# AbrahamSanders/realtime-codec-agent

Measured on NVIDIA B200. Metric: encode audio-sec/sec, higher is better.
Workload: dtype bf16

## Files before the change

realtime-codec-agent_b200/csrc/elementwise.cuh:

```cuda
#pragma once
#include "gemm_sm100.cuh"

namespace mc {

template <int KT>
__global__ void __launch_bounds__(256)
conv_first_kernel(const float* __restrict__ wav, long long ld, int T, int B, int T0, int s0, int C0,
                  const float* __restrict__ w , const float* __restrict__ bias,
                  __nv_bfloat16* __restrict__ out, int pad_rows) {
  pdl_launch_dependents();
  pdl_wait();
  const int cgroups = C0 / 8;
  const int cg = threadIdx.x % cgroups;
  const int slot = threadIdx.x / cgroups;
  const int frames_per_block = blockDim.x / cgroups;
  float wr[KT][8], br[8];
#pragma unroll
  for (int j = 0; j < KT; ++j) {
    const float4 a = __ldg(reinterpret_cast<const float4*>(w + j * C0 + cg * 8));
    const float4 c = __ldg(reinterpret_cast<const float4*>(w + j * C0 + cg * 8 + 4));
    wr[j][0] = a.x; wr[j][1] = a.y; wr[j][2] = a.z; wr[j][3] = a.w;
    wr[j][4] = c.x; wr[j][5] = c.y; wr[j][6] = c.z; wr[j][7] = c.w;
  }
#pragma unroll
// ... 78 lines not shown
#pragma unroll
    for (int u = 0; u < NV; ++u) ss += v[u].x * v[u].x + v[u].y * v[u].y + v[u].z * v[u].z + v[u].w * v[u].w;
#pragma unroll
    for (int o = 16; o > 0; o >>= 1) ss += __shfl_xor_sync(0xffffffffu, ss, o);
    const float inv = rsqrtf(ss / static_cast<float>(d) + eps);
    const int grp = row / grp_in;
    const long long obase = static_cast<long long>(grp) * grp_stride + grp_off + static_cast<long long>(row - grp * grp_in) * d;
    uint2* orow_p = reinterpret_cast<uint2*>(out + obase);
#pragma unroll
    for (int u = 0; u < NV; ++u) {
      uint2 o;
      o.x = pack_bf16x2(v[u].x * inv * g[u].x, v[u].y * inv * g[u].y);
      o.y = pack_bf16x2(v[u].z * inv * g[u].z, v[u].w * inv * g[u].w);
      orow_p[lane + 32 * u] = o;
    }
  }
}

__global__ void compact_rows_kernel(const float4* __restrict__ x, float4* __restrict__ y, int B, int r_in, int r_out,
                                    int d4) {
  pdl_launch_dependents();
  pdl_wait();
  const long long total = static_cast<long long>(B) * r_out * d4;
  for (long long idx = blockIdx.x * static_cast<long long>(blockDim.x) + threadIdx.x; idx < total;
       idx += static_cast<long long>(gridDim.x) * blockDim.x) {
    const int c = static_cast<int>(idx % d4);
    const long long row = idx / d4;
    const int j = static_cast<int>(row % r_out);
    const long long b = row / r_out;
    y[idx] = x[(b * r_in + (r_in - r_out) + j) * d4 + c];
  }
}

__global__ void gather_stem_kernel(const float4* __restrict__ stem, float4* __restrict__ x, int B, int F, int pre,
                                   int fstep, int d4) {
  pdl_launch_dependents();
  pdl_wait();
  const int per = F - pre;
  const long long total = static_cast<long long>(B) * per * d4;
  for (long long idx = blockIdx.x * static_cast<long long>(blockDim.x) + threadIdx.x; idx < total;
       idx += static_cast<long long>(gridDim.x) * blockDim.x) {
    const int c = static_cast<int>(idx % d4);
    const long long row = idx / d4;
    const int t = pre + static_cast<int>(row % per);
    const long long b = row / per;
    x[(b * F + t) * d4 + c] = __ldg(stem + (b * fstep + t) * d4 + c);
  }
}

__global__ void embed_codes_kernel(const long long* __restrict__ codes, const float* __restrict__ table ,
                                   int K, __nv_bfloat16* __restrict__ out, long long M) {
  pdl_launch_dependents();
  pdl_wait();
  const long long total = M * 8;
  for (long long idx = blockIdx.x * static_cast<long long>(blockDim.x) + threadIdx.x; idx < total;
       idx += static_cast<long long>(gridDim.x) * blockDim.x) {
    const long long m = idx >> 3;
    const int piece = static_cast<int>(idx & 7);
    uint4 o = make_uint4(0, 0, 0, 0);
    if (piece < 2) {
      long long code = codes[m];
      code = code < 0 ? 0 : (code >= K ? K - 1 : code);
      const float4* src = reinterpret_cast<const float4*>(table + code * 16 + piece * 8);
      const float4 a = __ldg(src), b = __ldg(src + 1);
      o.x = pack_bf16x2(a.x, a.y);
      o.y = pack_bf16x2(a.z, a.w);
      o.z = pack_bf16x2(b.x, b.y);
      o.w = pack_bf16x2(b.z, b.w);
    }
    *reinterpret_cast<uint4*>(out + m * 64 + piece * 8) = o;
  }
}

__global__ void pack_latents_kernel(const float* __restrict__ z , __nv_bfloat16* __restrict__ out,
                                    long long M) {
  const long long total = M * 8;
  for (long long idx = blockIdx.x * static_cast<long long>(blockDim.x) + threadIdx.x; idx < total;
       idx += static_cast<long long>(gridDim.x) * blockDim.x) {
    const long long m = idx >> 3;
// ... 129 lines not shown
```

realtime-codec-agent_b200/csrc/engine.cu:

```cuda
#include "engine_common.cuh"

#include "attn_sm100.cuh"
#include "attn_vq_simt.cuh"
#include "elementwise.cuh"
#include "gemm_sm100.cuh"
#include "gemm_splitk_sm100.cuh"
#include "ingest.cuh"
#include "post_sm100.cuh"
#include "vq_sm100.cuh"

using namespace mc;
using namespace mc_internal;

namespace {

struct GemmCall {
  const bf16* A; int64_t a_rows; int a_k_wrap;
  const bf16* W; const float* bias;
  int M, N, K, act, out_mode;
  void* out; int64_t ldo;
  int grp_in = INT_MAX, grp_valid = INT_MAX; int64_t grp_stride = 0, grp_off = 0;
  int rope_cols = 0, rope_period = 0, rope_offset = 0;
  int block_n = 0;
  const void* prefetch_ptr = nullptr;
// ... 238 lines not shown
  attention_window_simt_kernel<<<(unsigned)blocks, threads, 0, stream>>>(qkv, out, B, F, s.n_heads, s.window_left,
                                                                         s.window_right, out_rows, 0.125f);
  MC_LAUNCH_CHECK(h, "attention_window_simt_kernel");
  return MC_OK;
}

struct StackBufs {
  float* x;
  float* x2;
  bf16* hbuf;
  bf16* qkv;
  bf16* att;
  bf16* ffn;
  float* stats;
};

bool few_rows_regime(const mc_handle* h, long long M) {
  return (h->split_k == 2 || (h->split_k == 1 && h->in_session)) && M <= 2 * GEMM_BM;
}
bool fuse_norm_ok(const mc_handle* h, long long M) {
  if (h->spec.d_model % 64 != 0 || h->fuse_norm == 0) return false;
  return h->fuse_norm >= 2 || few_rows_regime(h, M);
}

int launch_rowstats(mc_handle* h, const float* x, const float* gamma, bf16* xb, float* stats, long long M, int d, cudaStream_t stream) {
  McProfScope prof(h, 3, 0.0, (double)M * d * 6.0, stream);
  mc_launch(h, rowstats_cast_kernel, dim3(ew_grid(h, M * (d / 64), 256)), dim3(256), 0, stream, x, gamma, xb, stats, M, d);
  MC_LAUNCH_CHECK(h, "rowstats_cast_kernel");
  return MC_OK;
}

int run_layers(mc_handle* h, const char* prefix, int n_layers, const StackBufs& b, int B, int F, int keep_rows,
               float** x_out, cudaStream_t stream, int fuse_mode = 0 ,
               const float* final_gamma = nullptr, bf16** xb_out = nullptr, float** stats_out = nullptr) {
  const mc_spec& s = h->spec;
  const int d = s.d_model, f = s.ffn_dim;
  const int nst = d / 64;
  const bool fused = fuse_mode == 1;
  const bool fused2 = fuse_mode != 0;
  std::vector<int> r_in(n_layers), r_out(n_layers);
  {
    int need = std::max(1, std::min(keep_rows, F));
    if (B == 1 && F <= GEMM_BM) need = F;
    for (int l = n_layers - 1; l >= 0; --l) {
      r_out[l] = need;
      need = (need >= F) ? F : std::min(F, need + s.window_left);
      if (!h->exact_cut && need < F) need = F - ((F - need) / 16) * 16;
      r_in[l] = need;
    }
  }
  float* x = b.x;
  float* xalt = b.x2;
  int rows = F;
  char name[128];
  for (int l = 0; l < n_layers; ++l) {
    auto T = [&](const char* leaf) {
      snprintf(name, sizeof(name), "%s.layers.%d.%s", prefix, l, leaf);
      return std::string(name);
    };
    const int Ri = rows, Ro = std::min(r_out[l], rows);
    const int Mi = B * Ri, Mo = B * Ro;
    if (!fused) MC_TRY(launch_rmsnorm(h, x, h->ptr<float>(T("norm1")), b.hbuf, Mi, d, INT_MAX, 0, 0, stream));
    GemmCall g{};
    if (fused) { g.row_stats = b.stats; g.row_stats_n = nst; }
    g.A = b.hbuf; g.a_rows = Mi; g.a_k_wrap = d; g.W = h->ptr<bf16>(T("wqkv")); g.bias = h->ptr<float>(T("bqkv"));
    g.M = Mi; g.N = 3 * d; g.K = d; g.act = ACT_NONE; g.out_mode = OUT_BF16; g.out = b.qkv; g.ldo = 3 * d;
    g.rope_cols = 2 * d; g.rope_period = Ri; g.rope_offset = F - Ri;
    g.prefetch_ptr = h->ptr<bf16>(T("wo")); g.prefetch_bytes = (long long)d * d * 2;
    MC_TRY(launch_gemm(h, g, stream));
    MC_TRY(launch_attention(h, b.qkv, b.att, B, Ri, Ro, (F - Ri) % 16, h->attn_impl, stream));
    if (Ro < Ri) {
      const long long items = (long long)Mo * (d / 4);
      McProfScope prof(h, 3, 0.0, (double)Mo * d * 8.0, stream);
      mc_launch(h, compact_rows_kernel, dim3(ew_grid(h, items, 256)), dim3(256), 0, stream, reinterpret_cast<const float4*>(x),
                reinterpret_cast<float4*>(xalt), B, Ri, Ro, d / 4);
      MC_LAUNCH_CHECK(h, "compact_rows_kernel");
      std::swap(x, xalt);
      rows = Ro;
    }
    GemmCall o{};
    o.A = b.att; o.a_rows = Mo; o.a_k_wrap = d; o.W = h->ptr<bf16>(T("wo")); o.bias = h->ptr<float>(T("bo"));
    o.M = Mo; o.N = d; o.K = d; o.act = ACT_NONE; o.out_mode = OUT_F32_RESIDUAL; o.out = x; o.ldo = d;
    o.prefetch_ptr = h->ptr<bf16>(T("w1")); o.prefetch_bytes = (long long)f * d * 2;
    if (fused2) { o.xb_out = b.hbuf; o.xb_gamma = h->ptr<float>(T("norm2")); o.stat_out = b.stats; }
    MC_TRY(launch_gemm(h, o, stream));
    if (!fused2) MC_TRY(launch_rmsnorm(h, x, h->ptr<float>(T("norm2")), b.hbuf, Mo, d, INT_MAX, 0, 0, stream));
    GemmCall u{};
    if (fused2) { u.row_stats = b.stats; u.row_stats_n = nst; }
    u.A = b.hbuf; u.a_rows = Mo; u.a_k_wrap = d; u.W = h->ptr<bf16>(T("w1")); u.bias = h->ptr<float>(T("b1"));
    u.M = Mo; u.N = f; u.K = d; u.act = ACT_GELU_TANH; u.out_mode = OUT_BF16; u.out = b.ffn; u.ldo = f;
    u.prefetch_ptr = h->ptr<bf16>(T("w2")); u.prefetch_bytes = (long long)d * f * 2;
    MC_TRY(launch_gemm(h, u, stream));
    GemmCall w{};
    w.A = b.ffn; w.a_rows = Mo; w.a_k_wrap = f; w.W = h->ptr<bf16>(T("w2")); w.bias = h->ptr<float>(T("b2"));
    w.M = Mo; w.N = d; w.K = f; w.act = ACT_NONE; w.out_mode = OUT_F32_RESIDUAL; w.out = x; w.ldo = d;
    if (l + 1 < n_layers) {
      snprintf(name, sizeof(name), "%s.layers.%d.wqkv", prefix, l + 1);
      w.prefetch_ptr = h->ptr<bf16>(name); w.prefetch_bytes = (long long)3 * d * d * 2;
    }
    if (fused) {
      const float* next_gamma = final_gamma;
      if (l + 1 < n_layers) {
// ... 140 lines not shown
  }
  return (int)dirty;
}

struct RaggedKeep {
  const int* rtable;
  int C, keep;
};

int encode_impl(mc_handle* h, const float* wav, int64_t ld, int B, int T, int keep, int64_t* codes, float* margin,
                float* z_e_out, cudaStream_t stream, const RaggedKeep* ragged = nullptr) {
  const mc_spec& s = h->spec;
  const int n = s.n_convs;
  int hop = 1;
  for (int i = 0; i < n; ++i) hop *= s.conv_strides[i];
  const int F = (T + hop - 1) / hop;
  if (F < 1) return h->fail(MC_ERR_ARG, "encode: empty input");
  if (F > s.max_positions) return h->fail(MC_ERR_ARG, "encode: %d frames exceed RoPE table (%d rows)", F, s.max_positions);
  if (keep <= 0 || keep > F) keep = F;
  const int Tp = F * hop;
  const int d = s.d_model, dq = s.codebook_dim;
  const long long Mll = (long long)B * F;
  if (Mll * std::max(3 * d, s.ffn_dim) > (long long)INT_MAX) return h->fail(MC_ERR_ARG, "encode: batch too large");
  const int M = (int)Mll;

  const int pre = stem_prefix_frames(s);
  const long long span_samples = (long long)(B - 1) * ld + T;
  const long long span_frames = span_samples / hop;
  const bool shared = h->shared_stem && B >= 2 && ld > 0 && ld < T && ld % hop == 0 && T % hop == 0 && F > pre &&
                      span_samples <= INT_MAX && span_frames + (long long)pre * B < (long long)B * F / 2;
  const int fuse_mode = !(fuse_norm_ok(h, Mll + B) && s.enc_layers > 0) ? 0 : ((h->fuse_norm == 3 && !few_rows_regime(h, Mll + B)) ? 2 : 1);
  const bool fused = fuse_mode == 1;
  const bool conv_producer = fused && few_rows_regime(h, Mll + B) && !shared;

  Carver cv;
  ConvPlan cp_full, cp_span, cp_pre;
  size_t ostem = 0;
  if (shared) {
    cp_span = plan_conv(s, cv, 1, (int)span_samples);
    cp_pre = plan_conv(s, cv, B, pre * hop);
    ostem = cv.take((size_t)span_frames * d * 4);
  } else {
    cp_full = plan_conv(s, cv, B, Tp);
  }
  Carver cv2 = cv;
  carve_stack(cv2, nullptr, M, d, s.ffn_dim, true);
  size_t oz = cv2.take((size_t)M * dq * 4);
  size_t ovq = cv2.take(vq_scratch_bytes(h, B * keep));
  const size_t ozg = ragged ? cv2.take((size_t)B * ragged->keep * dq * 4) : 0;
  MC_TRY(arena_reserve(h, cv2.off, stream));
  uint8_t* base = h->arena;
  StackBufs sb = carve_stack(cv, base, M, d, s.ffn_dim, false);
  float* z_e = reinterpret_cast<float*>(base + oz);
  void* vq_scratch = base + ovq;

  if (shared) {
    float* stem = reinterpret_cast<float*>(base + ostem);
    MC_TRY(run_conv_stack(h, cp_span, base, wav, span_samples, (int)span_samples, stem, 0, stream));
    MC_TRY(run_conv_stack(h, cp_pre, base, wav, ld, pre * hop, sb.x, (int64_t)F * d, stream));
    const long long items = (long long)B * (F - pre) * (d / 4);
    McProfScope prof(h, 3, 0.0, (double)B * (F - pre) * d * 8.0, stream);
    mc_launch(h, gather_stem_kernel, dim3(ew_grid(h, items, 256)), dim3(256), 0, stream, reinterpret_cast<const float4*>(stem),
              reinterpret_cast<float4*>(sb.x), B, F, pre, (int)(ld / hop), d / 4);
    MC_LAUNCH_CHECK(h, "gather_stem_kernel");
  } else {
    if (conv_producer)
      MC_TRY(run_conv_stack(h, cp_full, base, wav, ld, T, sb.x, (int64_t)F * d, stream, sb.hbuf, h->ptr<float>("enc.layers.0.norm1"), sb.stats));
    else
      MC_TRY(run_conv_stack(h, cp_full, base, wav, ld, T, sb.x, (int64_t)F * d, stream));
  }
  if (fused && !conv_producer) MC_TRY(launch_rowstats(h, sb.x, h->ptr<float>("enc.layers.0.norm1"), sb.hbuf, sb.stats, M, d, stream));
  const int keep_rows = z_e_out ? F : keep;
  float* xk = nullptr;
  bf16* xbk = sb.hbuf;
  float* stk = nullptr;
  MC_TRY(run_layers(h, "enc", s.enc_layers, sb, B, F, keep_rows, &xk, stream, fuse_mode, fused ? h->ptr<float>("enc.norm_f") : nullptr, &xbk, &stk));
  const int Mk = B * keep_rows;
  if (!fused) MC_TRY(launch_rmsnorm(h, xk, h->ptr<float>("enc.norm_f"), sb.hbuf, Mk, d, INT_MAX, 0, 0, stream));
  GemmCall pj{};
  if (fused) { pj.row_stats = stk; pj.row_stats_n = d / 64; }
  pj.A = fused ? xbk : sb.hbuf; pj.a_rows = Mk; pj.a_k_wrap = d; pj.W = h->ptr<bf16>("enc.proj.w"); pj.bias = h->ptr<float>("enc.proj.b");
  pj.M = Mk; pj.N = dq; pj.K = d; pj.act = ACT_NONE; pj.out_mode = OUT_F32; pj.out = z_e; pj.ldo = dq;
  MC_TRY(launch_gemm(h, pj, stream));
  if (z_e_out) MC_CUDA(h, cudaMemcpyAsync(z_e_out, z_e, (size_t)M * dq * 4, cudaMemcpyDeviceToDevice, stream));
  if (ragged) {
    float* zg = reinterpret_cast<float*>(base + ozg);
    pool_gather_rows_ragged_kernel<<<dim3(1, B), 256, 0, stream>>>(z_e, ragged->rtable, ragged->C, keep_rows, F, ragged->keep,
                                                                   dq, hop, zg);
    MC_LAUNCH_CHECK(h, "pool_gather_rows_ragged_kernel");
    return launch_vq(h, zg, B, ragged->keep, ragged->keep, codes, margin, vq_scratch, stream);
  }
  MC_TRY(launch_vq(h, z_e, B, keep_rows, keep, codes, margin, vq_scratch, stream));
  return MC_OK;
}

int decode_impl(mc_handle* h, const int64_t* codes, const float* z_q, int B, int F, int keep, float* wav,
                cudaStream_t stream) {
  const mc_spec& s = h->spec;
  const int n = s.n_convs;
  if (F < 1 || B < 1) return h->fail(MC_ERR_ARG, "decode: empty input");
  if (F > s.max_positions) return h->fail(MC_ERR_ARG, "decode: %d frames exceed RoPE table (%d rows)", F, s.max_positions);
  int hop = 1;
  for (int i = 0; i < n; ++i) hop *= s.conv_strides[i];
  const int d = s.d_model;
  const long long Mll = (long long)B * F;
  if (Mll * std::max(3 * d, s.ffn_dim) > (long long)INT_MAX) return h->fail(MC_ERR_ARG, "decode: batch too large");
  const int M = (int)Mll;
  const int total = F * hop;
  if (keep <= 0 || keep > total) keep = total;
// ... 338 lines not shown
}

int64_t mc_launch_count(const mc_handle* h) { return h ? h->launches : 0; }

int mc_profile_begin(mc_handle* h) {
  if (!h) return MC_ERR_ARG;
  for (auto& r : h->prof) { h->event_pool.push_back(r.a); h->event_pool.push_back(r.b); }
  h->prof.clear();
  h->profiling = true;
  return MC_OK;
}

int mc_profile_end(mc_handle* h, double* ms, double* flops, double* bytes, int64_t* launches, int32_t n_classes) {
  if (!h || !ms || !flops || !bytes || !launches) return MC_ERR_ARG;
  h->profiling = false;
  for (int c = 0; c < n_classes; ++c) { ms[c] = 0; flops[c] = 0; bytes[c] = 0; launches[c] = 0; }
  for (auto& r : h->prof) {
    cudaError_t e = cudaEventSynchronize(r.b);
    if (e != cudaSuccess) return h->fail(MC_ERR_CUDA, "mc_profile_end: %s", cudaGetErrorString(e));
    float t = 0.f;
    cudaEventElapsedTime(&t, r.a, r.b);
    if (r.cls < n_classes) { ms[r.cls] += t; flops[r.cls] += r.flops; bytes[r.cls] += r.bytes; launches[r.cls]++; }
    h->event_pool.push_back(r.a); h->event_pool.push_back(r.b);
  }
  h->prof.clear();
  return MC_OK;
}

int mc_set_option(mc_handle* h, const char* key, int32_t value) {
  if (!h || !key) return MC_ERR_ARG;
  const std::string k(key);
  if (k == "shared_stem") h->shared_stem = value != 0;
  else if (k == "exact_cut") { h->exact_cut = value != 0; h->tensor_gen++; }
  else if (k == "gemm_pair") h->gemm_pair = value != 0;
  else if (k == "fast_epilogue") h->fast_epilogue = value != 0;
  else if (k == "pdl") h->pdl = value != 0;
  else if (k == "attn_p_tmem") h->attn_p_tmem = value != 0;
  else if (k == "debug_repeat") h->debug_repeat = value;
  else if (k == "l2_prefetch") { h->l2_prefetch = value != 0; h->tensor_gen++; }
  else if (k == "fuse_norm") {
    if (value < 0 || value > 3) return h->fail(MC_ERR_ARG, "mc_set_option: fuse_norm is 0 .. 3");
    h->fuse_norm = value; h->tensor_gen++;
  }
  else if (k == "small_m_split_k") {
    if (value < 0 || value > 2) return h->fail(MC_ERR_ARG, "mc_set_option: small_m_split_k is 0, 1 or 2");
    h->split_k = value;
    h->tensor_gen++;
  }
  else if (k == "max_positions") {
    if (value < 1) return h->fail(MC_ERR_ARG, "mc_set_option: max_positions must be positive");
    h->spec.max_positions = value;
  }
  else return h->fail(MC_ERR_ARG, "mc_set_option: unknown option '%s'", key);
  return MC_OK;
}

int mc_set_debug_impl(mc_handle* h, int32_t attention_impl, int32_t vq_impl) {
  if (!h) return MC_ERR_ARG;
  h->gemm_pair = (attention_impl & 4) ? 0 : 1;
  attention_impl &= 1;
  h->attn_impl = attention_impl;
  h->vq_impl = vq_impl;
  return MC_OK;
}

int mc_op_gemm(mc_handle* h, const void* A, int64_t a_rows, int32_t a_k_wrap, const void* W, const float* bias,
// ... 909 lines not shown
```

realtime-codec-agent_b200/csrc/engine_common.cuh:

```cuda
#pragma once
#include <cuda.h>
#include <cuda_runtime.h>
#include <stdarg.h>
#include <stdio.h>
#include <string.h>

#include <algorithm>
#include <climits>
#include <map>
#include <set>
#include <string>
#include <tuple>
#include <unordered_map>
#include <utility>
#include <vector>

#include "../../include/magicodec_b200.h"
#include "ptx_sm100.cuh"

typedef __nv_bfloat16 bf16;

namespace mc_internal {

inline thread_local std::string g_create_error;
// ... 14 lines not shown
  }
  return fn;
}

struct Tensor {
  const void* p = nullptr;
  int64_t numel = 0;
};

}
using mc_internal::Tensor;

struct mc_handle {
  mc_spec spec{};
  int device = 0;
  int num_sms = 148;
  bool finalized = false;
  std::unordered_map<std::string, Tensor> tensors;
  std::string err;
  int64_t launches = 0;
  uint32_t tensor_gen = 0;
  int attn_impl = 0, vq_impl = 0;
  int gemm_pair = 1;
  bool fast_epilogue = true;
  bool attn_p_tmem = true;
  int split_k = 1;
  bool in_session = false;
  int debug_repeat = 1;
  int fuse_norm = 1;
  bool l2_prefetch = true;
  bool pdl = true;
  bool shared_stem = true;
  bool exact_cut = true;
  struct ProfRec { cudaEvent_t a, b; int cls; double flops; double bytes; };
  bool profiling = false;
  std::vector<ProfRec> prof;
  std::vector<cudaEvent_t> event_pool;
  std::set<const void*> smem_configured;
  uint8_t* arena = nullptr;
  size_t arena_cap = 0;
  size_t arena_off = 0;
  std::map<std::tuple<const void*, uint64_t, uint64_t, uint64_t, uint32_t, uint32_t>, CUtensorMap> maps;

  int fail(int code, const char* fmt, ...) {
    char buf[1024];
    va_list ap;
    va_start(ap, fmt);
    vsnprintf(buf, sizeof(buf), fmt, ap);
    va_end(ap);
    err = buf;
    return code;
  }
  const Tensor* find(const std::string& name) const {
    auto it = tensors.find(name);
    return it == tensors.end() ? nullptr : &it->second;
  }
  template <typename T>
  const T* ptr(const std::string& name) const {
    return reinterpret_cast<const T*>(tensors.at(name).p);
  }
};

#define MC_CUDA(h, expr)                                                                         \
  do {                                                                                           \
    cudaError_t e__ = (expr);                                                                    \
    if (e__ != cudaSuccess)                                                                      \
// ... 113 lines not shown
```

realtime-codec-agent_b200/csrc/gemm_sm100.cuh:

```cuda
#pragma once
#include <type_traits>

#include "ptx_sm100.cuh"

namespace mc {

enum : int { ACT_NONE = 0, ACT_GELU_TANH = 1 };
enum : int { OUT_BF16 = 0, OUT_F32 = 1, OUT_F32_RESIDUAL = 2 };

struct GemmParams {
  int M, N, K;
  int a_k_wrap;
  const float* bias;
  int act;
  int out_mode;
  void* out;
  long long ldo;
  int grp_in, grp_valid;
  long long grp_stride, grp_off;
  int tma_store;
  const float* rope_cos;
  int rope_ld;
  const float* rope_sin;
  int rope_cols;
// ... 26 lines not shown

constexpr int GEMM_BM = 128;
constexpr int GEMM_BK = 64;
constexpr int GEMM_THREADS = 256;
constexpr int kEpiBufBytes = 4096;

template <int BN>
struct GemmCfg {
  static constexpr int kStageBytesA = GEMM_BM * GEMM_BK * 2;
  static constexpr int kStageBytesB = BN * GEMM_BK * 2;
  static constexpr int kStageBytes = kStageBytesA + kStageBytesB;
  static constexpr int kStages = (BN == 256) ? 4 : (BN == 128 ? 6 : 8);
  static constexpr int kTmemCols = 2 * BN;
  static constexpr int kEpiBytes = 4 * 2 * kEpiBufBytes;
  static constexpr int kBarBytes = 256;
  static constexpr int kSmemBytes = kStages * kStageBytes + kEpiBytes + kBarBytes + 1024;
};

__device__ __forceinline__ float gelu_tanh_f(float x) {
  const float x2 = x * x;
  const float inner = fmaf(x2, 0.7978845608028654f * 0.044715f, 0.7978845608028654f);
  const float u = x * inner;
  float t;
  asm("tanh.approx.f32 %0, %1;" : "=f"(t) : "f"(u));
  const float hx = 0.5f * x;
  return fmaf(hx, t, hx);
}

__device__ __forceinline__ uint32_t pack_bf16x2(float lo, float hi) {
  __nv_bfloat162 h = __floats2bfloat162_rn(lo, hi);
  return *reinterpret_cast<uint32_t*>(&h);
}

struct EpiRegs {
  float bias[64];
  float rc[32], rs[32];
  int rope_pos = -1;
  int buf_sel = 0;
};

template <int BN>
__device__ __forceinline__ void epi_load_bias(const GemmParams& p, int n0, float (&b)[64]) {
#pragma unroll
  for (int j = 0; j < 64; j += 4) {
    float4 b4 = make_float4(0.f, 0.f, 0.f, 0.f);
    if (n0 + j < p.N) b4 = __ldg(reinterpret_cast<const float4*>(p.bias + n0 + j));
    b[j] = b4.x; b[j + 1] = b4.y; b[j + 2] = b4.z; b[j + 3] = b4.w;
  }
}

template <int BN, int RPW = 32>
__device__ __forceinline__ void gemm_epilogue_slab(const GemmParams& p, const CUtensorMap* map_out_p, uint32_t tmem_acc,
                                                   int row_base, int n_base, int q, int lane, uint8_t* my_bufs,
                                                   EpiRegs& st, uint64_t* ready_bar, uint32_t ready_parity) {
  const int g = row_base + q * RPW + (lane < RPW ? lane : 0);
  const int grp = g / p.grp_in;
  const int r = g - grp * p.grp_in;
  const bool row_ok = (lane < RPW) && (g < p.M) && (r < p.grp_valid);
  const long long obase = static_cast<long long>(grp) * p.grp_stride + p.grp_off + static_cast<long long>(r) * p.ldo;
  const bool has_bias = p.bias != nullptr;
  if (has_bias) epi_load_bias<BN>(p, n_base, st.bias);
  const float rs = (p.row_stats != nullptr && g < p.M) ? row_rs(p, g) : 1.0f;
  if (p.rope_period > 0) {
    const int pos = p.rope_offset + r % p.rope_period;
    if (pos != st.rope_pos) {
      st.rope_pos = pos;
// ... 10 lines not shown
#pragma unroll 1
  for (int c = 0; c < BN / 64; ++c) {
    const int n0 = n_base + c * 64;
    if (n0 >= p.N) break;
    uint32_t raw0[32], raw1[32];
    const uint32_t taddr = tmem_acc + (static_cast<uint32_t>(q * 32) << 16) + c * 64;
    tmem_ld_32x32b_x32(taddr, raw0);
    tmem_ld_32x32b_x32(taddr + 32, raw1);
    tmem_ld_wait();
    float v[64];
#pragma unroll
    for (int j = 0; j < 32; ++j) {
      v[j] = __uint_as_float(raw0[j]);
      v[32 + j] = __uint_as_float(raw1[j]);
    }
    if (p.row_stats != nullptr && has_bias) {
#pragma unroll
      for (int j = 0; j < 64; ++j) v[j] = fmaf(v[j], rs, st.bias[j]);
      if (c + 1 < BN / 64 && n0 + 64 < p.N) epi_load_bias<BN>(p, n0 + 64, st.bias);
    } else if (p.row_stats != nullptr) {
#pragma unroll
      for (int j = 0; j < 64; ++j) v[j] = __fmul_rn(v[j], rs);
    } else if (has_bias) {
#pragma unroll
      for (int j = 0; j < 64; ++j) v[j] += st.bias[j];
      if (c + 1 < BN / 64 && n0 + 64 < p.N) epi_load_bias<BN>(p, n0 + 64, st.bias);
    }
    if (p.act == ACT_GELU_TANH) {
#pragma unroll
      for (int j = 0; j < 64; ++j) v[j] = gelu_tanh_f(v[j]);
    }
    if (p.rope_period > 0 && n0 < p.rope_cols) {
#pragma unroll
      for (int j = 0; j < 32; ++j) {
        const float x1 = v[j], x2 = v[32 + j];
        v[j] = x1 * st.rc[j] - x2 * st.rs[j];
        v[32 + j] = x1 * st.rs[j] + x2 * st.rc[j];
      }
    }
    if (p.tma_store) {
      const int row0 = row_base + q * 32;
      const int sw = lane & 7;
      if (p.out_mode == OUT_BF16) {
        uint8_t* buf = my_bufs + st.buf_sel * kEpiBufBytes;
        if (lane == 0) tma_wait_group_read<1>();
        __syncwarp();
#pragma unroll
        for (int j = 0; j < 8; ++j) {
          uint4 w;
          w.x = pack_bf16x2(v[8 * j], v[8 * j + 1]);
          w.y = pack_bf16x2(v[8 * j + 2], v[8 * j + 3]);
          w.z = pack_bf16x2(v[8 * j + 4], v[8 * j + 5]);
          w.w = pack_bf16x2(v[8 * j + 6], v[8 * j + 7]);
          *reinterpret_cast<uint4*>(buf + lane * 128 + ((j ^ sw) << 4)) = w;
        }
        fence_proxy_async_smem();
        __syncwarp();
        if (lane == 0) {
          tma_store_2d(map_out_p, buf, n0, row0);
          tma_commit_group();
        }
        st.buf_sel ^= 1;
      } else {
#pragma unroll
        for (int half = 0; half < 2; ++half) {
          if (n0 + 32 * half < p.N) {
            uint8_t* buf = my_bufs + st.buf_sel * kEpiBufBytes;
            if (lane == 0) tma_wait_group_read<1>();
            __syncwarp();
#pragma unroll
            for (int j = 0; j < 8; ++j) {
// ... 125 lines not shown
#pragma unroll
  for (int j = 0; j < 32; ++j) {
    v[j] = __uint_as_float(lo[j]);
    v[32 + j] = __uint_as_float(hi[j]);
  }
  if (p.one != 0) {
#pragma unroll
    if (p.row_stats != nullptr) {
      const float rsc = st.row_scale;
#pragma unroll
      for (int j = 0; j < 32; j += 4) {
        const float4 b0 = lds_f4(sb + j);
        const float4 b1 = lds_f4(sb + 32 + j);
        v[j] = fmaf(v[j], rsc, b0.x); v[j + 1] = fmaf(v[j + 1], rsc, b0.y); v[j + 2] = fmaf(v[j + 2], rsc, b0.z); v[j + 3] = fmaf(v[j + 3], rsc, b0.w);
        v[32 + j] = fmaf(v[32 + j], rsc, b1.x); v[32 + j + 1] = fmaf(v[32 + j + 1], rsc, b1.y);
        v[32 + j + 2] = fmaf(v[32 + j + 2], rsc, b1.z); v[32 + j + 3] = fmaf(v[32 + j + 3], rsc, b1.w);
      }
    } else {
#pragma unroll
      for (int j = 0; j < 32; j += 4) {
        const float4 b0 = lds_f4(sb + j);
        const float4 b1 = lds_f4(sb + 32 + j);
        v[j] += b0.x; v[j + 1] += b0.y; v[j + 2] += b0.z; v[j + 3] += b0.w;
        v[32 + j] += b1.x; v[32 + j + 1] += b1.y; v[32 + j + 2] += b1.z; v[32 + j + 3] += b1.w;
      }
    }
    if (EPI == EPI_GELU_BF16) {
#pragma unroll
      for (int j = 0; j < 64; ++j) v[j] = gelu_tanh_f(v[j]);
    }
    if (EPI == EPI_ROPE_BF16) {
      if (n0 < p.rope_cols) {
#pragma unroll
        for (int j = 0; j < 32; ++j) {
          const float x1 = v[j], x2 = v[32 + j];
          v[j] = x1 * st.rc[j] - x2 * st.rs[j];
          v[32 + j] = x1 * st.rs[j] + x2 * st.rc[j];
        }
      }
    }
  }
  const int sw = lane & 7;
  if (EPI == EPI_RESID_F32) {
#pragma unroll
    for (int half = 0; half < 2; ++half) {
      uint8_t* buf = my_bufs + st.buf_sel * kEpiBufBytes;
      if (lane == 0) tma_wait_group_read<1>();
      __syncwarp();
#pragma unroll
      for (int j = 0; j < 8; ++j) {
        const float* vv = v + 32 * half + 4 * j;
        sts_u4(buf + lane * 128 + ((j ^ sw) << 4), make_uint4(__float_as_uint(vv[0]), __float_as_uint(vv[1]), __float_as_uint(vv[2]),
                                                               __float_as_uint(vv[3])));
      }
      fence_proxy_async_smem();
      __syncwarp();
      if (lane == 0) {
        tma_reduce_add_2d(map_out_p, buf, n0 + 32 * half, row0);
        tma_commit_group();
      }
      st.buf_sel ^= 1;
    }
  } else {
    uint8_t* buf = my_bufs + st.buf_sel * kEpiBufBytes;
    if (lane == 0) tma_wait_group_read<1>();
    __syncwarp();
#pragma unroll
    for (int j = 0; j < 8; ++j) {
      uint4 w;
      w.x = pack_bf16x2(v[8 * j], v[8 * j + 1]);
      w.y = pack_bf16x2(v[8 * j + 2], v[8 * j + 3]);
// ... 488 lines not shown
```

realtime-codec-agent_b200/csrc/gemm_splitk_sm100.cuh:

```cuda
#pragma once
#include "gemm_sm100.cuh"

namespace mc {

template <int BN>
struct GemmSkCfg {
  static constexpr int kStages = 4;
  static constexpr int kStageBytesA = GEMM_BM * GEMM_BK * 2;
  static constexpr int kStageBytesB = BN * GEMM_BK * 2;
  static constexpr int kStageBytes = kStageBytesA + kStageBytesB;
  static constexpr int kPartBytes = GEMM_BM * BN * 4;
  static constexpr int kTmemCols = BN < 32 ? 32 : BN;
  static constexpr int kBarBytes = 256;
  static constexpr int kSmemBytes = kStages * kStageBytes + kBarBytes + 1024;
  static_assert(kPartBytes <= kStages * kStageBytes, "partial tile must fit in the stage ring");
  static_assert(kSmemBytes <= 113 * 1024, "two CTAs per SM");
};

__device__ __forceinline__ float4 ld_dsmem_f4(uint32_t cluster_addr) {
  float4 v;
  asm volatile("ld.shared::cluster.v4.f32 {%0, %1, %2, %3}, [%4];" : "=f"(v.x), "=f"(v.y), "=f"(v.z), "=f"(v.w) : "r"(cluster_addr));
  return v;
}

// ... 179 lines not shown
      for (int hf = 0; hf < 2; ++hf) {
#pragma unroll
        for (int q = 0; q < kHalf / 4; ++q) {
          const int chunk = (hf * 32 + e_c0 + q * 4) >> 2;
          const uint32_t a = prow + ((chunk ^ sw) << 4);
          float4 parts[S];
#pragma unroll
          for (int s = 0; s < S; ++s) parts[s] = ld_dsmem_f4(mapa_shared(a, s));
          float4 acc = parts[0];
#pragma unroll
          for (int s = 1; s < S; ++s) { acc.x += parts[s].x; acc.y += parts[s].y; acc.z += parts[s].z; acc.w += parts[s].w; }
          v[hf][q * 4] = acc.x; v[hf][q * 4 + 1] = acc.y; v[hf][q * 4 + 2] = acc.z; v[hf][q * 4 + 3] = acc.w;
        }
      }
      if (p.row_stats != nullptr) {
#pragma unroll
        for (int hf = 0; hf < 2; ++hf)
#pragma unroll
          for (int j = 0; j < kHalf; ++j) v[hf][j] = p.bias != nullptr ? fmaf(v[hf][j], e_rs, e_bias[hf][j]) : __fmul_rn(v[hf][j], e_rs);
      } else if (p.bias != nullptr) {
#pragma unroll
        for (int hf = 0; hf < 2; ++hf)
#pragma unroll
          for (int j = 0; j < kHalf; ++j) v[hf][j] += e_bias[hf][j];
      }
      if (p.act == ACT_GELU_TANH) {
#pragma unroll
        for (int hf = 0; hf < 2; ++hf)
#pragma unroll
          for (int j = 0; j < kHalf; ++j) v[hf][j] = gelu_tanh_f(v[hf][j]);
      }
      if (p.rope_period > 0 && n0 < p.rope_cols) {
#pragma unroll
        for (int j = 0; j < kHalf; ++j) {
          const float x1 = v[0][j], x2 = v[1][j];
          v[0][j] = x1 * e_cos[j] - x2 * e_sin[j];
          v[1][j] = x1 * e_sin[j] + x2 * e_cos[j];
        }
      }
#pragma unroll
      for (int hf = 0; hf < 2; ++hf) {
#pragma unroll
        for (int q = 0; q < kHalf / 4; ++q) {
          const int n = n0 + hf * 32 + e_c0 + q * 4;
          if (n >= p.N) continue;
          const float* vv = &v[hf][q * 4];
          if (p.out_mode == OUT_BF16) {
            uint2 w;
            w.x = pack_bf16x2(vv[0], vv[1]);
            w.y = pack_bf16x2(vv[2], vv[3]);
            *reinterpret_cast<uint2*>(reinterpret_cast<__nv_bfloat16*>(p.out) + e_obase + n) = w;
          } else {
            float4 x = make_float4(vv[0], vv[1], vv[2], vv[3]);
            if (p.out_mode == OUT_F32_RESIDUAL) {
              const float* old = &e_xold[hf][q * 4];
              x.x += old[0]; x.y += old[1]; x.z += old[2]; x.w += old[3];
            }
            *reinterpret_cast<float4*>(reinterpret_cast<float*>(p.out) + e_obase + n) = x;
            if (p.xb_out != nullptr) {
              const float* ga = &e_gamma[hf][q * 4];
              ss = fmaf(x.x, x.x, ss); ss = fmaf(x.y, x.y, ss); ss = fmaf(x.z, x.z, ss); ss = fmaf(x.w, x.w, ss);
              uint2 w;
              w.x = pack_bf16x2(x.x * ga[0], x.y * ga[1]);
              w.y = pack_bf16x2(x.z * ga[2], x.w * ga[3]);
              *reinterpret_cast<uint2*>(p.xb_out + e_orow * p.N + n) = w;
            }
          }
        }
      }
    }
    if (p.xb_out != nullptr) {
// ... 17 lines not shown
```

Before: 5627.

## Share layer-0 QKV projection across overlapping windows via a deduplicated stem table

When windows share a stem, the first encoder layer's rmsnorm and QKV GEMM now run once over the deduplicated table of span frames plus per-batch prefix rows, instead of over B*F rows. A new expand kernel applies RoPE per absolute position and scatters the results into the per-window qkv buffer in bf16. The gather kernel now builds x from the same unified table. This trades a smaller GEMM for an extra f32 qtab round trip and a scatter kernel. The rope math is unified into an fma-based helper, which may change rounding slightly.

```diff
diff --git a/realtime-codec-agent_b200/csrc/elementwise.cuh b/realtime-codec-agent_b200/csrc/elementwise.cuh
--- a/realtime-codec-agent_b200/csrc/elementwise.cuh
+++ b/realtime-codec-agent_b200/csrc/elementwise.cuh
@@ -134,19 +134,102 @@
   }
 }
 
-__global__ void gather_stem_kernel(const float4* __restrict__ stem, float4* __restrict__ x, int B, int F, int pre,
-                                   int fstep, int d4) {
-  pdl_launch_dependents();
-  pdl_wait();
-  const int per = F - pre;
-  const long long total = static_cast<long long>(B) * per * d4;
+__device__ __forceinline__ long long stem_table_row(int b, int t, int pre, int fstep, long long span_rows) {
+  return t < pre ? span_rows + static_cast<long long>(b) * pre + t : static_cast<long long>(b) * fstep + t;
+}
+
+__global__ void gather_stem_kernel(const float4* __restrict__ tab, float4* __restrict__ x, int B, int F, int pre,
+                                   int fstep, long long span_rows, int d4) {
+  pdl_launch_dependents();
+  pdl_wait();
+  const long long total = static_cast<long long>(B) * F * d4;
   for (long long idx = blockIdx.x * static_cast<long long>(blockDim.x) + threadIdx.x; idx < total;
        idx += static_cast<long long>(gridDim.x) * blockDim.x) {
     const int c = static_cast<int>(idx % d4);
     const long long row = idx / d4;
-    const int t = pre + static_cast<int>(row % per);
-    const long long b = row / per;
-    x[(b * F + t) * d4 + c] = __ldg(stem + (b * fstep + t) * d4 + c);
+    const int t = static_cast<int>(row % F);
+    const int b = static_cast<int>(row / F);
+    x[idx] = __ldg(tab + stem_table_row(b, t, pre, fstep, span_rows) * d4 + c);
+  }
+}
+
+constexpr int kExpandSmemPositions = 192;
+
+template <bool kSmemAngles>
+__global__ void __launch_bounds__(256)
+qkv_rope_expand_kernel(const float* __restrict__ qtab, const float* __restrict__ rope_cos, const float* __restrict__ rope_sin,
+                       int rope_ld, __nv_bfloat16* __restrict__ qkv, int B, int F, int pre, int fstep, long long span_rows,
+                       int d) {
+  extern __shared__ float4 s_ang[];
+  pdl_launch_dependents();
+  if (kSmemAngles) {
+    float* sa = reinterpret_cast<float*>(s_ang);
+    for (int i = threadIdx.x; i < 64 * F; i += blockDim.x) {
+      const int t = i >> 6, j = i & 63;
+      sa[i] = j < 32 ? __ldg(rope_cos + static_cast<long long>(j) * rope_ld + t)
+                     : __ldg(rope_sin + static_cast<long long>(j - 32) * rope_ld + t);
+    }
+    __syncthreads();
+  }
+  pdl_wait();
+  const int n3 = 3 * d, per_row = n3 / 16, rope_items = d / 8;
+  const long long total = (span_rows + static_cast<long long>(B) * pre) * per_row;
+  for (long long idx = blockIdx.x * static_cast<long long>(blockDim.x) + threadIdx.x; idx < total;
+       idx += static_cast<long long>(gridDim.x) * blockDim.x) {
+    const long long r = idx / per_row;
+    const int it = static_cast<int>(idx - r * per_row);
+    const bool rot = it < rope_items;
+    const int j0 = rot ? ((it >> 2) << 6) + ((it & 3) << 3) : 2 * d + ((it - rope_items) << 4);
+    const int j1 = j0 + (rot ? 32 : 8);
+    float a[8], c[8];
+    {
+      const float4* s0 = reinterpret_cast<const float4*>(qtab + r * n3 + j0);
+      const float4* s1 = reinterpret_cast<const float4*>(qtab + r * n3 + j1);
+      const float4 a0 = __ldg(s0), a1 = __ldg(s0 + 1), c0 = __ldg(s1), c1 = __ldg(s1 + 1);
+      a[0] = a0.x; a[1] = a0.y; a[2] = a0.z; a[3] = a0.w; a[4] = a1.x; a[5] = a1.y; a[6] = a1.z; a[7] = a1.w;
+      c[0] = c0.x; c[1] = c0.y; c[2] = c0.z; c[3] = c0.w; c[4] = c1.x; c[5] = c1.y; c[6] = c1.z; c[7] = c1.w;
+    }
+    long long off;
+    int step, b_lo, b_hi;
+    if (r < span_rows) {
+      off = r; step = fstep;
+      b_lo = r < F ? 0 : static_cast<int>((r - F) / fstep + 1);
+      b_hi = r < pre ? -1 : static_cast<int>(min(static_cast<long long>(B - 1), (r - pre) / fstep));
+    } else {
+      off = r - span_rows; step = pre;
+      b_lo = b_hi = static_cast<int>(off / pre);
+    }
+    for (int b = b_lo; b <= b_hi; ++b) {
+      const int t = static_cast<int>(off - static_cast<long long>(b) * step);
+      float y0[8], y1[8];
+      if (rot) {
+        const int jh = j0 & 63;
+        float cs[8], sn[8];
+        if (kSmemAngles) {
+          const float4* p = s_ang + t * 16 + (jh >> 2);
+          const float4 c0 = p[0], c1 = p[1], s0 = p[8], s1 = p[9];
+          cs[0] = c0.x; cs[1] = c0.y; cs[2] = c0.z; cs[3] = c0.w; cs[4] = c1.x; cs[5] = c1.y; cs[6] = c1.z; cs[7] = c1.w;
+          sn[0] = s0.x; sn[1] = s0.y; sn[2] = s0.z; sn[3] = s0.w; sn[4] = s1.x; sn[5] = s1.y; sn[6] = s1.z; sn[7] = s1.w;
+        } else {
+#pragma unroll
+          for (int i = 0; i < 8; ++i) {
+            cs[i] = __ldg(rope_cos + static_cast<long long>(jh + i) * rope_ld + t);
+            sn[i] = __ldg(rope_sin + static_cast<long long>(jh + i) * rope_ld + t);
+          }
+        }
+#pragma unroll
+        for (int i = 0; i < 8; ++i) rope_rotate(a[i], c[i], cs[i], sn[i], y0[i], y1[i]);
+      } else {
+#pragma unroll
+        for (int i = 0; i < 8; ++i) { y0[i] = a[i]; y1[i] = c[i]; }
+      }
+      __nv_bfloat16* o = qkv + (static_cast<long long>(b) * F + t) * n3;
+      uint4 w;
+      w.x = pack_bf16x2(y0[0], y0[1]); w.y = pack_bf16x2(y0[2], y0[3]); w.z = pack_bf16x2(y0[4], y0[5]); w.w = pack_bf16x2(y0[6], y0[7]);
+      *reinterpret_cast<uint4*>(o + j0) = w;
+      w.x = pack_bf16x2(y1[0], y1[1]); w.y = pack_bf16x2(y1[2], y1[3]); w.z = pack_bf16x2(y1[4], y1[5]); w.w = pack_bf16x2(y1[6], y1[7]);
+      *reinterpret_cast<uint4*>(o + j1) = w;
+    }
   }
 }
 
diff --git a/realtime-codec-agent_b200/csrc/engine.cu b/realtime-codec-agent_b200/csrc/engine.cu
--- a/realtime-codec-agent_b200/csrc/engine.cu
+++ b/realtime-codec-agent_b200/csrc/engine.cu
@@ -294,7 +294,8 @@
 
 int run_layers(mc_handle* h, const char* prefix, int n_layers, const StackBufs& b, int B, int F, int keep_rows,
                float** x_out, cudaStream_t stream, int fuse_mode = 0 ,
-               const float* final_gamma = nullptr, bf16** xb_out = nullptr, float** stats_out = nullptr) {
+               const float* final_gamma = nullptr, bf16** xb_out = nullptr, float** stats_out = nullptr,
+               bool qkv0_ready = false) {
   const mc_spec& s = h->spec;
   const int d = s.d_model, f = s.ffn_dim;
   const int nst = d / 64;
@@ -322,14 +323,16 @@
     };
     const int Ri = rows, Ro = std::min(r_out[l], rows);
     const int Mi = B * Ri, Mo = B * Ro;
-    if (!fused) MC_TRY(launch_rmsnorm(h, x, h->ptr<float>(T("norm1")), b.hbuf, Mi, d, INT_MAX, 0, 0, stream));
-    GemmCall g{};
-    if (fused) { g.row_stats = b.stats; g.row_stats_n = nst; }
-    g.A = b.hbuf; g.a_rows = Mi; g.a_k_wrap = d; g.W = h->ptr<bf16>(T("wqkv")); g.bias = h->ptr<float>(T("bqkv"));
-    g.M = Mi; g.N = 3 * d; g.K = d; g.act = ACT_NONE; g.out_mode = OUT_BF16; g.out = b.qkv; g.ldo = 3 * d;
-    g.rope_cols = 2 * d; g.rope_period = Ri; g.rope_offset = F - Ri;
-    g.prefetch_ptr = h->ptr<bf16>(T("wo")); g.prefetch_bytes = (long long)d * d * 2;
-    MC_TRY(launch_gemm(h, g, stream));
+    if (!(l == 0 && qkv0_ready)) {
+      if (!fused) MC_TRY(launch_rmsnorm(h, x, h->ptr<float>(T("norm1")), b.hbuf, Mi, d, INT_MAX, 0, 0, stream));
+      GemmCall g{};
+      if (fused) { g.row_stats = b.stats; g.row_stats_n = nst; }
+      g.A = b.hbuf; g.a_rows = Mi; g.a_k_wrap = d; g.W = h->ptr<bf16>(T("wqkv")); g.bias = h->ptr<float>(T("bqkv"));
+      g.M = Mi; g.N = 3 * d; g.K = d; g.act = ACT_NONE; g.out_mode = OUT_BF16; g.out = b.qkv; g.ldo = 3 * d;
+      g.rope_cols = 2 * d; g.rope_period = Ri; g.rope_offset = F - Ri;
+      g.prefetch_ptr = h->ptr<bf16>(T("wo")); g.prefetch_bytes = (long long)d * d * 2;
+      MC_TRY(launch_gemm(h, g, stream));
+    }
     MC_TRY(launch_attention(h, b.qkv, b.att, B, Ri, Ro, (F - Ri) % 16, h->attn_impl, stream));
     if (Ro < Ri) {
       const long long items = (long long)Mo * (d / 4);
@@ -536,6 +539,8 @@
   const int fuse_mode = !(fuse_norm_ok(h, Mll + B) && s.enc_layers > 0) ? 0 : ((h->fuse_norm == 3 && !few_rows_regime(h, Mll + B)) ? 2 : 1);
   const bool fused = fuse_mode == 1;
   const bool conv_producer = fused && few_rows_regime(h, Mll + B) && !shared;
+  const long long tab_rows = shared ? span_frames + (long long)B * pre : 0;
+  const bool shared_qkv = shared && h->shared_qkv && !fused && s.enc_layers > 0 && !few_rows_regime(h, tab_rows);
 
   Carver cv;
   ConvPlan cp_full, cp_span, cp_pre;
@@ -543,7 +548,7 @@
   if (shared) {
     cp_span = plan_conv(s, cv, 1, (int)span_samples);
     cp_pre = plan_conv(s, cv, B, pre * hop);
-    ostem = cv.take((size_t)span_frames * d * 4);
+    ostem = cv.take((size_t)tab_rows * d * 4);
   } else {
     cp_full = plan_conv(s, cv, B, Tp);
   }
@@ -552,20 +557,24 @@
   size_t oz = cv2.take((size_t)M * dq * 4);
   size_t ovq = cv2.take(vq_scratch_bytes(h, B * keep));
   const size_t ozg = ragged ? cv2.take((size_t)B * ragged->keep * dq * 4) : 0;
+  const size_t qtab_bytes = (size_t)tab_rows * 3 * d * 4;
+  const bool qtab_in_ffn = qtab_bytes <= (size_t)M * s.ffn_dim * 2;
+  const size_t oqtab = shared_qkv && !qtab_in_ffn ? cv2.take(qtab_bytes) : 0;
   MC_TRY(arena_reserve(h, cv2.off, stream));
   uint8_t* base = h->arena;
   StackBufs sb = carve_stack(cv, base, M, d, s.ffn_dim, false);
   float* z_e = reinterpret_cast<float*>(base + oz);
   void* vq_scratch = base + ovq;
 
+  float* stem = shared ? reinterpret_cast<float*>(base + ostem) : nullptr;
+  const int fstep = (int)(ld / hop);
   if (shared) {
-    float* stem = reinterpret_cast<float*>(base + ostem);
     MC_TRY(run_conv_stack(h, cp_span, base, wav, span_samples, (int)span_samples, stem, 0, stream));
-    MC_TRY(run_conv_stack(h, cp_pre, base, wav, ld, pre * hop, sb.x, (int64_t)F * d, stream));
-    const long long items = (long long)B * (F - pre) * (d / 4);
-    McProfScope prof(h, 3, 0.0, (double)B * (F - pre) * d * 8.0, stream);
+    MC_TRY(run_conv_stack(h, cp_pre, base, wav, ld, pre * hop, stem + (size_t)span_frames * d, (int64_t)pre * d, stream));
+    const long long items = (long long)B * F * (d / 4);
+    McProfScope prof(h, 3, 0.0, (double)B * F * d * 8.0, stream);
     mc_launch(h, gather_stem_kernel, dim3(ew_grid(h, items, 256)), dim3(256), 0, stream, reinterpret_cast<const float4*>(stem),
-              reinterpret_cast<float4*>(sb.x), B, F, pre, (int)(ld / hop), d / 4);
+              reinterpret_cast<float4*>(sb.x), B, F, pre, fstep, span_frames, d / 4);
     MC_LAUNCH_CHECK(h, "gather_stem_kernel");
   } else {
     if (conv_producer)
@@ -574,11 +583,30 @@
       MC_TRY(run_conv_stack(h, cp_full, base, wav, ld, T, sb.x, (int64_t)F * d, stream));
   }
   if (fused && !conv_producer) MC_TRY(launch_rowstats(h, sb.x, h->ptr<float>("enc.layers.0.norm1"), sb.hbuf, sb.stats, M, d, stream));
+  if (shared_qkv) {
+    float* qtab = qtab_in_ffn ? reinterpret_cast<float*>(sb.ffn) : reinterpret_cast<float*>(base + oqtab);
+    MC_TRY(launch_rmsnorm(h, stem, h->ptr<float>("enc.layers.0.norm1"), sb.hbuf, (int)tab_rows, d, INT_MAX, 0, 0, stream));
+    GemmCall g{};
+    g.A = sb.hbuf; g.a_rows = tab_rows; g.a_k_wrap = d; g.W = h->ptr<bf16>("enc.layers.0.wqkv"); g.bias = h->ptr<float>("enc.layers.0.bqkv");
+    g.M = (int)tab_rows; g.N = 3 * d; g.K = d; g.act = ACT_NONE; g.out_mode = OUT_F32; g.out = qtab; g.ldo = 3 * d;
+    MC_TRY(launch_gemm(h, g, stream));
+    const long long items = tab_rows * (3 * d / 16);
+    McProfScope prof(h, 3, 0.0, (double)tab_rows * 3 * d * 4.0 + (double)M * 3 * d * 2.0, stream);
+    const int grid = (int)std::min<long long>((items + 255) / 256, (long long)h->num_sms * 4);
+    if (F <= kExpandSmemPositions)
+      mc_launch(h, qkv_rope_expand_kernel<true>, dim3(grid), dim3(256), (size_t)F * 64 * 4, stream, qtab, h->ptr<float>("rope.cos"),
+                h->ptr<float>("rope.sin"), s.max_positions, sb.qkv, B, F, pre, fstep, span_frames, d);
+    else
+      mc_launch(h, qkv_rope_expand_kernel<false>, dim3(grid), dim3(256), 0, stream, qtab, h->ptr<float>("rope.cos"),
+                h->ptr<float>("rope.sin"), s.max_positions, sb.qkv, B, F, pre, fstep, span_frames, d);
+    MC_LAUNCH_CHECK(h, "qkv_rope_expand_kernel");
+  }
   const int keep_rows = z_e_out ? F : keep;
   float* xk = nullptr;
   bf16* xbk = sb.hbuf;
   float* stk = nullptr;
-  MC_TRY(run_layers(h, "enc", s.enc_layers, sb, B, F, keep_rows, &xk, stream, fuse_mode, fused ? h->ptr<float>("enc.norm_f") : nullptr, &xbk, &stk));
+  MC_TRY(run_layers(h, "enc", s.enc_layers, sb, B, F, keep_rows, &xk, stream, fuse_mode, fused ? h->ptr<float>("enc.norm_f") : nullptr, &xbk, &stk,
+                    shared_qkv));
   const int Mk = B * keep_rows;
   if (!fused) MC_TRY(launch_rmsnorm(h, xk, h->ptr<float>("enc.norm_f"), sb.hbuf, Mk, d, INT_MAX, 0, 0, stream));
   GemmCall pj{};
@@ -983,6 +1011,7 @@
   const std::string k(key);
   if (k == "shared_stem") h->shared_stem = value != 0;
   else if (k == "exact_cut") { h->exact_cut = value != 0; h->tensor_gen++; }
+  else if (k == "shared_qkv") h->shared_qkv = value != 0;
   else if (k == "gemm_pair") h->gemm_pair = value != 0;
   else if (k == "fast_epilogue") h->fast_epilogue = value != 0;
   else if (k == "pdl") h->pdl = value != 0;
diff --git a/realtime-codec-agent_b200/csrc/engine_common.cuh b/realtime-codec-agent_b200/csrc/engine_common.cuh
--- a/realtime-codec-agent_b200/csrc/engine_common.cuh
+++ b/realtime-codec-agent_b200/csrc/engine_common.cuh
@@ -70,6 +70,7 @@
   bool pdl = true;
   bool shared_stem = true;
   bool exact_cut = true;
+  bool shared_qkv = true;
   struct ProfRec { cudaEvent_t a, b; int cls; double flops; double bytes; };
   bool profiling = false;
   std::vector<ProfRec> prof;
diff --git a/realtime-codec-agent_b200/csrc/gemm_sm100.cuh b/realtime-codec-agent_b200/csrc/gemm_sm100.cuh
--- a/realtime-codec-agent_b200/csrc/gemm_sm100.cuh
+++ b/realtime-codec-agent_b200/csrc/gemm_sm100.cuh
@@ -82,6 +82,11 @@
   return *reinterpret_cast<uint32_t*>(&h);
 }
 
+__device__ __forceinline__ void rope_rotate(float x1, float x2, float c, float s, float& y1, float& y2) {
+  y1 = __fmaf_rn(x1, c, -__fmul_rn(x2, s));
+  y2 = __fmaf_rn(x1, s, __fmul_rn(x2, c));
+}
+
 struct EpiRegs {
   float bias[64];
   float rc[32], rs[32];
@@ -158,11 +163,7 @@
     }
     if (p.rope_period > 0 && n0 < p.rope_cols) {
 #pragma unroll
-      for (int j = 0; j < 32; ++j) {
-        const float x1 = v[j], x2 = v[32 + j];
-        v[j] = x1 * st.rc[j] - x2 * st.rs[j];
-        v[32 + j] = x1 * st.rs[j] + x2 * st.rc[j];
-      }
+      for (int j = 0; j < 32; ++j) rope_rotate(v[j], v[32 + j], st.rc[j], st.rs[j], v[j], v[32 + j]);
     }
     if (p.tma_store) {
       const int row0 = row_base + q * 32;
@@ -354,11 +355,7 @@
     if (EPI == EPI_ROPE_BF16) {
       if (n0 < p.rope_cols) {
 #pragma unroll
-        for (int j = 0; j < 32; ++j) {
-          const float x1 = v[j], x2 = v[32 + j];
-          v[j] = x1 * st.rc[j] - x2 * st.rs[j];
-          v[32 + j] = x1 * st.rs[j] + x2 * st.rc[j];
-        }
+        for (int j = 0; j < 32; ++j) rope_rotate(v[j], v[32 + j], st.rc[j], st.rs[j], v[j], v[32 + j]);
       }
     }
   }
diff --git a/realtime-codec-agent_b200/csrc/gemm_splitk_sm100.cuh b/realtime-codec-agent_b200/csrc/gemm_splitk_sm100.cuh
--- a/realtime-codec-agent_b200/csrc/gemm_splitk_sm100.cuh
+++ b/realtime-codec-agent_b200/csrc/gemm_splitk_sm100.cuh
@@ -235,11 +235,7 @@
       }
       if (p.rope_period > 0 && n0 < p.rope_cols) {
 #pragma unroll
-        for (int j = 0; j < kHalf; ++j) {
-          const float x1 = v[0][j], x2 = v[1][j];
-          v[0][j] = x1 * e_cos[j] - x2 * e_sin[j];
-          v[1][j] = x1 * e_sin[j] + x2 * e_cos[j];
-        }
+        for (int j = 0; j < kHalf; ++j) rope_rotate(v[0][j], v[1][j], e_cos[j], e_sin[j], v[0][j], v[1][j]);
       }
 #pragma unroll
       for (int hf = 0; hf < 2; ++hf) {
```

After: 5773, median of 6. 1.03x the previous value.
